# scomup/point-cloud-registration

Measured on AMD Instinct MI355X. Metric: M-correspondences/sec, plane calc_H_g_e2 on the B-01 stand-in (1.06 M pts), higher is better.
Workload: dtype f32; 1 GPU; plane_b01; kind=plane, target_points=1060000, scan_points_per_gpu=1060000, parallelism=scan-shard x1, devices_visible=1, scan_points_job=1060000, gauss_newton_iters_to_converge=5, correspondences_last_step=1060000

## Files before the change

### include/pcr.h

```cpp
#ifndef PCR_H
#define PCR_H

#include <stdint.h>

#ifdef __cplusplus
extern "C" {
#endif

#define PCR_API __attribute__((visibility("default")))

#define PCR_ABI_VERSION 5

typedef int pcr_status;
enum {
    PCR_OK = 0,
    PCR_ERR_INVALID = -1,
    PCR_ERR_HIP = -2,
    PCR_ERR_NO_TARGET = -3,
    PCR_ERR_COMM = -4,
    PCR_ERR_SINGULAR = -5,
    PCR_ERR_NOMEM = -6,
    PCR_ERR_UNSUPPORTED = -7
};

// ... 275 lines not shown
PCR_API pcr_status pcr_fgr_solo_max(pcr_context *ctx, int64_t *m_max);

#define PCR_COMPAT_M_MAX 32768
#define PCR_COMPAT_K_MAX 64
PCR_API pcr_status pcr_compat_bits(pcr_context *ctx, const float *src, const float *dst, int64_t m, double d,
                                   uint64_t *bits );
PCR_API pcr_status pcr_compat_degrees(pcr_context *ctx, const float *src, const float *dst, int64_t m, double d, int64_t *deg1 ,
                                      int64_t *deg2 );
PCR_API pcr_status pcr_compat_consensus(pcr_context *ctx, const float *src, const float *dst, int64_t m, double d, int n_seeds, int k,
                                        int64_t *deg1_or_null , int64_t *deg2_or_null , int32_t *seeds ,
                                        int32_t *members , int32_t *scores , int *n_seeds_out);

enum { PCR_K_LINEARIZE = 0, PCR_K_FINALIZE = 1, PCR_K_NN = 2, PCR_K_REDUCE = 3, PCR_K_ALLREDUCE = 4, PCR_K_CERTIFY = 5, PCR_K_COUNT = 6 };
PCR_API pcr_status pcr_profile_enable(pcr_context *ctx, int on);
PCR_API pcr_status pcr_profile_reset(pcr_context *ctx);
PCR_API pcr_status pcr_profile_read(pcr_context *ctx, int64_t launches[PCR_K_COUNT], double total_ms[PCR_K_COUNT]);
PCR_API pcr_status pcr_profile_read_n(pcr_context *ctx, int capacity, int64_t *launches, double *total_ms, int *count);
PCR_API pcr_status pcr_target_index_info(pcr_target *t, double *cell, int64_t dims[3], int64_t *occupied, int64_t *n);
PCR_API pcr_status pcr_target_index_population(pcr_target *t, int64_t *pop_max, int64_t *pop_p99, int *heavy);
PCR_API pcr_status pcr_target_index_x_order(pcr_target *t, double *xq);
PCR_API int pcr_x_order_rule(int f32_point_target, int heavy, int64_t n, int cell_bits);
PCR_API pcr_status pcr_target_index_halo(pcr_target *t, double *halo, int64_t *records);
PCR_API pcr_status pcr_target_index_halo2(pcr_target *t, double *halo, int64_t *records);
PCR_API pcr_status pcr_target_filter_band(pcr_target *t, double *band);
PCR_API pcr_status pcr_nn_counters(pcr_target *t, pcr_scan *s, const double T[16], double max_dist, double out[11]);
PCR_API pcr_status pcr_nn_counters_x(pcr_target *t, pcr_scan *s, const double T[16], double max_dist, double out[3]);
PCR_API pcr_status pcr_nn_counters_edge(pcr_target *t, pcr_scan *s, const double T[16], double max_dist, double out[9]);
PCR_API pcr_status pcr_set_variant(pcr_context *ctx, int variant);
PCR_API pcr_status pcr_get_variant(pcr_context *ctx, int *variant);
PCR_API pcr_status pcr_set_nn_mode(pcr_context *ctx, int mode);
PCR_API pcr_status pcr_set_reuse(pcr_context *ctx, int mode, double tau, double mu);
PCR_API pcr_status pcr_get_reuse(pcr_context *ctx, int *mode, double *tau, double *mu);
PCR_API pcr_status pcr_scan_reuse_stats(pcr_scan *s, double out[8]);
PCR_API pcr_status pcr_set_fuse_finalize(pcr_context *ctx, int on);
PCR_API int pcr_has_dev_kernels(void);
PCR_API pcr_status pcr_get_pipeline(pcr_context *ctx, int *variant, int *fuse_finalize, int *nn_mode);

#ifdef __cplusplus
}
#endif
#endif
```

### point_cloud_registration_amd/_capi.py

```python

import atexit
import ctypes as C
import os
import weakref

import numpy as np

_HERE = os.path.dirname(os.path.abspath(__file__))
LIB_PATH = os.environ.get("PCR_LIB") or os.path.join(_HERE, "libpcr_hip.so")
DEV_LIB_PATH = os.path.join(_HERE, "libpcr_hip_dev.so")

PCR_OK = 0
PCR_ERR_INVALID, PCR_ERR_HIP, PCR_ERR_NO_TARGET, PCR_ERR_COMM, PCR_ERR_SINGULAR, PCR_ERR_NOMEM = -1, -2, -3, -4, -5, -6
PCR_ERR_UNSUPPORTED = -7
ICP, PLANE, VPLANE, NDT = 0, 1, 2, 3
FLAG_ICP_RR_QUIRK = 1
FLAG_NO_SCAN_SORT = 2
FLAG_LOCAL_ONLY = 4
FLAG_HOST_LOOP = 8
FLAG_DEVICE_LOOP = 16
FLAG_KEEP_ORDER = 32
K_LINEARIZE, K_FINALIZE, K_NN, K_REDUCE, K_ALLREDUCE, K_CERTIFY, K_COUNT = 0, 1, 2, 3, 4, 5, 6
KERNEL_NAMES = ("linearize", "finalize", "nn", "reduce", "allreduce", "certify")
NN_FULL, NN_TRACK, NN_LIST = 0, 1, 2
# ... 66 lines not shown
    "pcr_ransac_poses": (C.c_int, [_vp, _f32p, _f32p, C.c_int64, C.c_int64, C.c_uint64, C.c_float, C.c_float, C.c_float,
                                   C.POINTER(C.c_int64), _f32p, C.POINTER(C.c_int32), C.POINTER(C.c_int64), _vp, _vp, _vp]),
    "pcr_pose_score_splits": (C.c_int, [C.c_int64, C.c_int64]),
    "pcr_fgr_linearize": (C.c_int, [_vp, _f32p, _f32p, C.c_int64, _vp, _f64p, C.c_double, _f64p, _vp]),
    "pcr_fgr_pose": (C.c_int, [_vp, _f32p, _f32p, C.c_int64, _vp, _f64p, C.c_double, C.c_double, C.c_double, C.c_int, C.c_int,
                               C.c_double, C.c_uint, _f64p, C.POINTER(C.c_int), C.POINTER(C.c_int), C.POINTER(C.c_double), _vp, _vp]),
    "pcr_fgr_tuples": (C.c_int, [_vp, _f32p, _f32p, C.c_int64, C.c_int64, C.c_uint64, C.c_float, C.c_float, _vp,
                                 C.POINTER(C.c_int64)]),
    "pcr_fgr_blocks": (C.c_int, [C.c_int64]),
    "pcr_fgr_solo_max": (C.c_int, [_vp, C.POINTER(C.c_int64)]),
    "pcr_compat_bits": (C.c_int, [_vp, _f32p, _f32p, C.c_int64, C.c_double, _vp]),
    "pcr_compat_degrees": (C.c_int, [_vp, _f32p, _f32p, C.c_int64, C.c_double, _vp, _vp]),
    "pcr_compat_consensus": (C.c_int, [_vp, _f32p, _f32p, C.c_int64, C.c_double, C.c_int, C.c_int, _vp, _vp, _vp, _vp, _vp,
                                       C.POINTER(C.c_int)]),
    "pcr_profile_enable": (C.c_int, [_vp, C.c_int]),
    "pcr_profile_reset": (C.c_int, [_vp]),
    "pcr_profile_read": (C.c_int, [_vp, _i64p, _f64p]),
    "pcr_target_index_info": (C.c_int, [_vp, C.POINTER(C.c_double), _i64p, C.POINTER(C.c_int64), C.POINTER(C.c_int64)]),
    "pcr_target_index_halo": (C.c_int, [_vp, C.POINTER(C.c_double), C.POINTER(C.c_int64)]),
    "pcr_target_index_population": (C.c_int, [_vp, C.POINTER(C.c_int64), C.POINTER(C.c_int64), C.POINTER(C.c_int)]),
    "pcr_target_index_x_order": (C.c_int, [_vp, C.POINTER(C.c_double)]),
    "pcr_x_order_rule": (C.c_int, [C.c_int, C.c_int, C.c_int64, C.c_int]),
    "pcr_set_variant": (C.c_int, [_vp, C.c_int]),
    "pcr_get_variant": (C.c_int, [_vp, C.POINTER(C.c_int)]),
    "pcr_set_nn_mode": (C.c_int, [_vp, C.c_int]),
    "pcr_set_fuse_finalize": (C.c_int, [_vp, C.c_int]),
    "pcr_get_pipeline": (C.c_int, [_vp, C.POINTER(C.c_int), C.POINTER(C.c_int), C.POINTER(C.c_int)]),
    "pcr_nn_counters": (C.c_int, [_vp, _vp, _f64p, C.c_double, _f64p]),
    "pcr_nn_counters_x": (C.c_int, [_vp, _vp, _f64p, C.c_double, _f64p]),
    "pcr_nn_counters_edge": (C.c_int, [_vp, _vp, _f64p, C.c_double, _f64p]),
    "pcr_set_reuse": (C.c_int, [_vp, C.c_int, C.c_double, C.c_double]),
    "pcr_get_reuse": (C.c_int, [_vp, C.POINTER(C.c_int), C.POINTER(C.c_double), C.POINTER(C.c_double)]),
    "pcr_scan_reuse_stats": (C.c_int, [_vp, _f64p]),
    "pcr_hash64": (C.c_int, [_vp, C.c_uint64, C.POINTER(C.c_uint64)]),
    "pcr_target_filter_band": (C.c_int, [_vp, C.POINTER(C.c_double)]),
    "pcr_target_index_halo2": (C.c_int, [_vp, C.POINTER(C.c_double), C.POINTER(C.c_int64)]),
    "pcr_usable_cpus": (C.c_int, []),
    "pcr_has_dev_kernels": (C.c_int, []),
    "pcr_abi_version": (C.c_int, []),
    "pcr_context_trim": (C.c_int, [_vp, C.POINTER(C.c_uint64)]),
    "pcr_profile_read_n": (C.c_int, [_vp, C.c_int, _i64p, _f64p, C.POINTER(C.c_int)]),
    "pcr_scan_read_matches": (C.c_int, [_vp, _vp]),
    "pcr_comm_p2p_finegrained": (C.c_int, [_vp, C.POINTER(C.c_int)]),
    "pcr_lzf_decompress": (C.c_int, [_vp, C.c_uint64, _vp, C.c_uint64, C.POINTER(C.c_uint64)]),
    "pcr_lzf_compress": (C.c_int, [_vp, C.c_uint64, _vp, C.c_uint64, C.POINTER(C.c_uint64)]),
    "pcr_gn_set": (C.c_int, [_vp, _vp, C.c_int, _vp, C.c_int, C.c_int64, C.c_int, _f64p]),
    "pcr_coreset": (C.c_int, [_vp, _f64p, C.c_int, C.c_int64, _f64p, C.c_int, C.c_int64, C.POINTER(C.c_int64), _f64p, _i64p,
                              _f64p]),
    "pcr_linearize_rows": (C.c_int, [_vp, _vp, C.c_int, _f64p, C.c_double, C.c_uint, _vp, _vp, _vp, _vp, _vp]),
    "pcr_linearize_weighted": (C.c_int, [_vp, _vp, C.c_int, _f64p, C.c_double, C.c_uint, _f64p, _f64p]),
    "pcr_scan_coreset": (C.c_int, [_vp, _vp, C.c_int, _f64p, C.c_double, C.c_uint, C.c_int, C.c_int64, _i64p, _f64p,
                                   C.POINTER(C.c_int64)]),
    "pcr_target_estimate_covariances": (C.c_int, [_vp, C.c_int, C.c_int, C.c_double, _vp]),
    "pcr_target_set_covariances": (C.c_int, [_vp, _f32p]),
    "pcr_target_get_covariances": (C.c_int, [_vp, _f32p]),
    "pcr_scan_estimate_covariances": (C.c_int, [_vp, C.c_int, C.c_int, C.c_double, _vp]),
    "pcr_scan_set_covariances": (C.c_int, [_vp, _f32p]),
    "pcr_scan_get_covariances": (C.c_int, [_vp, _f32p]),
    "pcr_gicp_linearize": (C.c_int, [_vp, _vp, _f64p, C.c_double, C.c_uint, _f64p]),
    "pcr_gicp_align": (C.c_int, [_vp, _vp, _f64p, C.c_int, C.c_double, C.c_double, C.c_uint, _f64p, C.POINTER(C.c_int), _vp]),
    "pcr_scan_estimate_normals": (C.c_int, [_vp, C.c_int, _vp]),
    "pcr_scan_set_normals": (C.c_int, [_vp, _f32p]),
    "pcr_scan_get_normals": (C.c_int, [_vp, _f32p]),
    "pcr_symm_linearize": (C.c_int, [_vp, _vp, _f64p, C.c_double, C.c_double, C.c_uint, _f64p]),
    "pcr_symm_align": (C.c_int, [_vp, _vp, _f64p, C.c_int, C.c_double, C.c_double, C.c_double, C.c_uint, _f64p, C.POINTER(C.c_int), _vp]),
    "pcr_target_set_intensity": (C.c_int, [_vp, _f32p, _vp]),
# ... 194 lines not shown

    def synchronize(self):
        check(lib().pcr_context_synchronize(self.handle))

    def stream(self):
        s = _vp()
        check(lib().pcr_context_stream(self.handle, C.byref(s)))
        return s.value

    def set_variant(self, v):
        check(lib().pcr_set_variant(self.handle, int(v)))

    def get_variant(self):
        v = C.c_int(0)
        check(lib().pcr_get_variant(self.handle, C.byref(v)))
        return v.value

    def set_nn_mode(self, m):
        check(lib().pcr_set_nn_mode(self.handle, int(m)))

    def set_fuse_finalize(self, on):
        check(lib().pcr_set_fuse_finalize(self.handle, int(bool(on))))

    def set_reuse(self, mode=None, tau=0.0, mu=0.0):
        if mode is None:
            mode = self.get_reuse()["mode"]
        check(lib().pcr_set_reuse(self.handle, int(mode), float(tau), float(mu)))

    def get_reuse(self):
        m, t, u = C.c_int(0), C.c_double(0), C.c_double(0)
        check(lib().pcr_get_reuse(self.handle, C.byref(m), C.byref(t), C.byref(u)))
        return {"mode": m.value, "tau": t.value, "mu": u.value}

    def get_pipeline(self):
        v, f, m = C.c_int(0), C.c_int(0), C.c_int(0)
        check(lib().pcr_get_pipeline(self.handle, C.byref(v), C.byref(f), C.byref(m)))
        return {"variant": v.value, "fuse_finalize": f.value, "nn_mode": m.value, "reuse": self.get_reuse()["mode"]}

    def pipeline(self, variant=None, fuse_finalize=None, nn_mode=None, reuse=None):
        import contextlib

        @contextlib.contextmanager
        def _cm():
            prev = self.get_pipeline()
            try:
                if variant is not None:
                    self.set_variant(variant)
                if fuse_finalize is not None:
                    self.set_fuse_finalize(fuse_finalize)
                if nn_mode is not None:
                    self.set_nn_mode(nn_mode)
                if reuse is not None:
                    self.set_reuse(reuse)
                yield self
            finally:
                errs = []
                for fn, val in ((self.set_variant, prev["variant"]), (self.set_fuse_finalize, prev["fuse_finalize"]),
                                (self.set_nn_mode, prev["nn_mode"]), (self.set_reuse, prev["reuse"])):
                    try:
                        fn(val)
                    except Exception as exc:
                        errs.append(exc)
                import sys as _sys
                if errs and _sys.exc_info()[0] is None:
                    raise errs[0]
        return _cm()
# ... 1196 lines not shown
```

### point_cloud_registration_amd/csrc/api.hip

```cpp
#include <math.h>
#include <stdarg.h>
#include <stdlib.h>
#include <string.h>

#include <string>

#include "gn_math.h"
#include "pcr_internal.h"

static thread_local std::string g_last_error;

void pcr_set_error(const char *fmt, ...) {
    char buf[1024];
    va_list ap;
    va_start(ap, fmt);
    vsnprintf(buf, sizeof buf, fmt, ap);
    va_end(ap);
    g_last_error = buf;
}

extern "C" const char *pcr_last_error(void) { return g_last_error.c_str(); }
extern "C" const char *pcr_version(void) { return "pcr-hip 0.4 (gfx950)"; }
extern "C" int pcr_abi_version(void) { return PCR_ABI_VERSION; }

// ... 133 lines not shown
    pcr_context *ctx = new pcr_context();
    ctx->device = device;
    ctx->num_cu = prop.multiProcessorCount > 0 ? prop.multiProcessorCount : 256;
    ctx->stream = stream;
    ctx->variant = 2;
    const char *v = getenv("PCR_VARIANT");
    if (v && *v) { const int vv = atoi(v); ctx->variant = vv == 0 ? 0 : (vv == 1 ? 1 : 2); }
    const char *nm = getenv("PCR_NN_MODE");
    if (nm && *nm) {
        const int m = atoi(nm);
#ifdef PCR_DEV
        if (m == 0 || m == 2 || m == 3 || m == 4) ctx->nn_mode = m;
#else
        if (m == 0 || m == 3) ctx->nn_mode = m;
#endif
        else fprintf(stderr, "[pcr] PCR_NN_MODE=%s is not a search mode of this library (0, 3; developer build: 2, 4): using 0\n", nm);
    }
#ifdef PCR_DEV
    const char *ff = getenv("PCR_FUSE_FINALIZE");
    if (ff && *ff) ctx->fuse_finalize = atoi(ff) != 0;
#endif
    const char *lf = getenv("PCR_LOCAL_FRAC");
    if (lf && *lf) ctx->local_frac = atof(lf);
    const char *cm = getenv("PCR_VOXEL_CELL_MULT");
    if (cm && atof(cm) > 0) ctx->voxel_cell_mult = atof(cm);
    const char *vf = getenv("PCR_VOX_FILTER");
    if (vf && *vf) ctx->vox_filter = atoi(vf) != 0;
    const char *fa = getenv("PCR_FILTER_AFTER");
    if (fa && *fa) ctx->filter_after = atoi(fa);
    const char *vo = getenv("PCR_VOX_OCC");
    if (vo && *vo) ctx->vox_occ = atoi(vo) != 0;
    const char *tl = getenv("PCR_TILE_LOCAL");
    if (tl && *tl) ctx->tile_local = atoi(tl) != 0;
    const char *sd = getenv("PCR_STALL_DEBUG");
    if (sd && *sd) ctx->stall_debug = atoi(sd) != 0;
    const char *rp = getenv("PCR_RETIRE_PERIOD");
    if (rp && *rp) ctx->retire_period = atoi(rp);
    const char *ru = getenv("PCR_REUSE");
    if (ru && *ru) ctx->reuse = atoi(ru);
    const char *rt = getenv("PCR_REUSE_TAU");
    if (rt && *rt) ctx->reuse_tau = atof(rt);
    const char *rm = getenv("PCR_REUSE_MU");
    if (rm && *rm) ctx->reuse_mu = atof(rm);
    if (ctx->reuse < 0 || ctx->reuse > 2) ctx->reuse = 0;
    const char *cl = getenv("PCR_CACHE_LIMIT_MB");
    if (cl && *cl && atof(cl) >= 0) ctx->cache_limit = (size_t)(atof(cl) * 1048576.0);
    *out = ctx;
    return PCR_OK;
}

extern "C" pcr_status pcr_context_destroy(pcr_context *ctx) {
    if (!ctx) return PCR_OK;
    (void)hipSetDevice(ctx->device);
    (void)hipStreamSynchronize(ctx->stream);
    pcr_comm_destroy(ctx);
    pcr_cache_clear(ctx);
    for (auto &e : ctx->prof_events) { (void)hipEventDestroy(e.start); (void)hipEventDestroy(e.stop); }
    for (auto &e : ctx->prof_free) { (void)hipEventDestroy(e.start); (void)hipEventDestroy(e.stop); }
    if (ctx->d_partials) (void)hipFree(ctx->d_partials);
    if (ctx->d_out) (void)hipFree(ctx->d_out);
    if (ctx->h_out) (void)hipHostFree(ctx->h_out);
    if (ctx->h_batch) (void)hipHostFree(ctx->h_batch);
    if (ctx->d_pose) (void)hipFree(ctx->d_pose);
    if (ctx->d_trace) (void)hipFree(ctx->d_trace);
    if (ctx->d_tile_ctr) (void)hipFree(ctx->d_tile_ctr);
    (void)hipStreamDestroy(ctx->stream);
    delete ctx;
    return PCR_OK;
}

extern "C" pcr_status pcr_context_trim(pcr_context *ctx, uint64_t *released_bytes) {
    PCR_REQUIRE(ctx, "ctx is NULL");
    HIP_TRY(hipSetDevice(ctx->device));
    HIP_TRY(hipStreamSynchronize(ctx->stream));
    size_t before;
    { CacheLock lock(ctx->cache_mu); before = ctx->cache_bytes; }
    pcr_cache_clear(ctx);
    if (released_bytes) *released_bytes = (uint64_t)before;
    return PCR_OK;
}

extern "C" pcr_status pcr_context_stream(pcr_context *ctx, void **stream) {
    PCR_REQUIRE(ctx && stream, "NULL argument");
    *stream = (void *)ctx->stream;
    return PCR_OK;
}

extern "C" pcr_status pcr_context_synchronize(pcr_context *ctx) {
    PCR_REQUIRE(ctx, "ctx is NULL");
    HIP_TRY(hipStreamSynchronize(ctx->stream));
    return PCR_OK;
}

extern "C" pcr_status pcr_set_variant(pcr_context *ctx, int variant) {
// ... 50 lines not shown

extern "C" pcr_status pcr_set_nn_mode(pcr_context *ctx, int mode) {
    PCR_REQUIRE(ctx, "ctx is NULL");
    PCR_REQUIRE(mode == 0 || (mode >= 2 && mode <= 4), "nn mode must be 0, 2, 3 or 4");
#ifndef PCR_DEV
    PCR_REQUIRE(mode != 2 && mode != 4, "the wave-cooperative searches (2: LDS-staged, 4: MFMA-filtered) are in the developer build only (make dev: libpcr_hip_dev.so)");
#endif
    ctx->nn_mode = mode;
    return PCR_OK;
}

extern "C" pcr_status pcr_set_reuse(pcr_context *ctx, int mode, double tau, double mu) {
    PCR_REQUIRE(ctx, "ctx is NULL");
    PCR_REQUIRE(mode >= 0 && mode <= 2, "reuse mode must be 0 (off), 1 (automatic) or 2 (forced)");
    ctx->reuse = mode;
    if (tau > 0) ctx->reuse_tau = tau;
    if (mu > 0) ctx->reuse_mu = mu;
    return PCR_OK;
}

extern "C" pcr_status pcr_get_reuse(pcr_context *ctx, int *mode, double *tau, double *mu) {
    PCR_REQUIRE(ctx, "ctx is NULL");
    if (mode) *mode = ctx->reuse;
    if (tau) *tau = ctx->reuse_tau;
    if (mu) *mu = ctx->reuse_mu;
    return PCR_OK;
}

extern "C" pcr_status pcr_scan_reuse_stats(pcr_scan *s, double out[8]) {
    PCR_REQUIRE(s && out, "NULL argument");
    out[0] = (double)s->st_passes[0]; out[1] = (double)s->st_passes[1]; out[2] = (double)s->st_passes[2];
    out[3] = (double)s->st_marked; out[4] = (double)s->st_listed_of;
    out[5] = (double)s->last_mode; out[6] = (double)s->last_marked; out[7] = s->last_motion;
    return PCR_OK;
}

#include <dlfcn.h>
static struct {
    int state;
    int (*push)(const char *);
    int (*pop)();
} g_roctx;

static bool roctx_on() {
    if (g_roctx.state == 0) {
        g_roctx.state = -1;
        const char *e = getenv("PCR_ROCTX");
        if (e && atoi(e) != 0) {
            const char *names[] = {"libroctx64.so.4", "libroctx64.so", "/opt/rocm/lib/libroctx64.so"};
            void *lib = nullptr;
            for (const char *n : names) { lib = dlopen(n, RTLD_NOW | RTLD_LOCAL); if (lib) break; }
            if (lib) {
                g_roctx.push = (int (*)(const char *))dlsym(lib, "roctxRangePushA");
                g_roctx.pop = (int (*)())dlsym(lib, "roctxRangePop");
                if (g_roctx.push && g_roctx.pop) g_roctx.state = 1;
            }
        }
    }
    return g_roctx.state == 1;
}
void pcr_roctx_push(const char *name) { if (roctx_on()) (void)g_roctx.push(name); }
void pcr_roctx_pop() { if (roctx_on()) (void)g_roctx.pop(); }

void pcr_prof_begin(pcr_context *ctx, int kernel, ProfEvent *ev) {
    ev->kernel = -1;
    if (!ctx->prof_on || !ctx->prof_this_pass) return;
// ... 583 lines not shown
```

### point_cloud_registration_amd/csrc/gn_math.h

```cpp
#pragma once

#include <math.h>

#if defined(__HIPCC__)
#define PCR_HD __host__ __device__
#else
#define PCR_HD
#endif

PCR_HD static inline int gn_solve6(double (*A)[7], const double H[36], const double g[6], double x[6]) {
#pragma unroll
    for (int i = 0; i < 6; ++i) {
#pragma unroll
        for (int j = 0; j < 6; ++j) A[i][j] = H[6 * i + j];
        A[i][6] = g[i];
    }
    int singular = 0;
#pragma unroll
    for (int c = 0; c < 6; ++c) {
        int piv = c;
        double pmax = fabs(A[c][c]);
#pragma unroll
        for (int r = c + 1; r < 6; ++r) { const double v = fabs(A[r][c]); if (v > pmax) { pmax = v; piv = r; } }
        if (pmax == 0.0) singular = 1;
// ... 111 lines not shown
    for (int k = 0; k < 7; ++k) {
        double p[3] = {(double)c[0], (double)c[1], (double)c[2]};
        if (k > 0) { const int ax = (k - 1) >> 1; p[ax] += ((k - 1) & 1) ? (double)e[ax] : -(double)e[ax]; }
        double d2 = 0;
        for (int i = 0; i < 3; ++i) {
            const double a = Ta[4 * i] * p[0] + Ta[4 * i + 1] * p[1] + Ta[4 * i + 2] * p[2] + Ta[4 * i + 3];
            const double b = Tb[4 * i] * p[0] + Tb[4 * i + 1] * p[1] + Tb[4 * i + 2] * p[2] + Tb[4 * i + 3];
            d2 += (b - a) * (b - a);
        }
        sum += sqrt(d2);
    }
    return sum / 7.0;
}

PCR_HD static inline int gn_choose_nn_mode(int reuse, int have_prev, int track_valid, double motion, double prev_motion,
                                           double tau_len) {
    if (reuse == 0 || !have_prev) return 0;
    if (reuse == 2) return track_valid ? 2 : 1;
    if (!(motion < tau_len)) return 0;
    if (track_valid) return 2;
    if (motion == 0.0) return 1;
    if (prev_motion >= 0.0 && prev_motion < 8.0 * tau_len && motion > 0.3 * prev_motion) return 1;
    return 0;
}

PCR_HD static inline double gn_filter_band(double maxabs) {
    return 1.7321 * 1.01 * maxabs * 5.9604644775390625e-8 + 1e-30;
}
PCR_HD static inline void gn_filter_bounds(double band, double bound, float *bound2_ff, float *mu_ff) {
    const double bf = (bound + band) * 1.00002;
    *bound2_ff = (float)(bf * bf * 1.000001);
    *mu_ff = (float)(2.0 * band + 3e-5 * bf);
}
```

### point_cloud_registration_amd/csrc/pass.hip

```cpp
#include <stdlib.h>

#include "pass_device.h"

static int grid8(int64_t want, int64_t cap = INT64_MAX) {
    int64_t nb = (want + 7) & ~(int64_t)7;
    if (nb > (cap & ~(int64_t)7)) nb = cap & ~(int64_t)7;
    return nb < 8 ? 8 : (int)nb;
}

static double cell_edge(const pcr_target *t) { return t->is_voxel ? t->gd.h : (double)t->gf.h; }

pcr_status pcr_ensure_scratch(pcr_context *ctx, int64_t n_points) {
    (void)n_points;
    if (!ctx->d_partials) {
        ctx->max_blocks = (ctx->num_cu * 16 + 7) & ~7;
        HIP_TRY(pcr_malloc_retry((void **)&ctx->d_partials, sizeof(double) * 32 * (size_t)(ctx->max_blocks + 8)));
        HIP_TRY(pcr_malloc_retry((void **)&ctx->d_out, sizeof(double) * 32));
        HIP_TRY(pcr_malloc_retry((void **)&ctx->d_pose, sizeof(PoseDev)));
        HIP_TRY(hipHostMalloc(&ctx->h_out, sizeof(double) * 64, hipHostMallocMapped | hipHostMallocCoherent));
        memset(ctx->h_out, 0, sizeof(double) * 64);
        HIP_TRY(hipHostGetDevicePointer((void **)&ctx->h_out_dev, ctx->h_out, 0));
        const size_t ctr_words = 9 * PCR_TICKET_STRIDE + (size_t)PCR_TILE_CTRS * PCR_TILE_STRIDE + 16;
        HIP_TRY(pcr_malloc_retry((void **)&ctx->d_tile_ctr, sizeof(uint32_t) * ctr_words));
        HIP_TRY(hipMemsetAsync(ctx->d_tile_ctr, 0, sizeof(uint32_t) * ctr_words, ctx->stream));
        auto blocks_per_cu = [](int which, int fallback) { const int nb = nn_blocks_per_cu(which); return nb > 0 ? nb : fallback; };
#ifdef PCR_DEV
        ctx->nn_blocks_per_cu[4] = blocks_per_cu(PCR_OCC_MFMA, 2);
        ctx->nn_blocks_per_cu[2] = pcr_dev_coop_blocks_per_cu();
#endif
        ctx->nn_blocks_lb = blocks_per_cu(PCR_OCC_POINT_LB, 4);
        ctx->nn_blocks_per_cu[0] = blocks_per_cu(PCR_OCC_POINT, 4);
        ctx->nn_blocks_per_cu[1] = blocks_per_cu(PCR_OCC_VOXEL, 4);
        ctx->nn_blocks_per_cu[3] = blocks_per_cu(PCR_OCC_FILTER, 4);
    }
    return PCR_OK;
}

static int64_t blocks_wanted(const pcr_context *ctx, int64_t n) {
    const int64_t want = (n + 255) / 256, cap = (int64_t)ctx->num_cu * 8;
    return want < cap ? want : cap;
}
int choose_blocks(const pcr_context *ctx, int64_t n) { return grid8(blocks_wanted(ctx, n), ctx->max_blocks); }

struct Pass {
    pcr_context *ctx;
    pcr_target *t;
    pcr_scan *s;
    int kind;
    LinArgs a;
    FinArgs f;
    bool one_kernel;
    bool fused_fin;
    bool gn_inline;
    double motion;
// ... 361 lines not shown
static pcr_status wait_host_word(pcr_context *ctx, Pred ready, const char *what) {
    for (long spin = 0; spin < 4000000L; ++spin) {
        if (ready()) { __atomic_thread_fence(__ATOMIC_ACQUIRE); return PCR_OK; }
        __builtin_ia32_pause();
    }
    HIP_TRY(hipStreamSynchronize(ctx->stream));
    if (!ready()) { pcr_set_error("%s did not report completion", what); return PCR_ERR_HIP; }
    __atomic_thread_fence(__ATOMIC_ACQUIRE);
    return PCR_OK;
}

static void retire_completed(pcr_context *ctx) {
    if (ctx->retire_period > 0 && ++ctx->passes_since_query >= (uint32_t)ctx->retire_period) {
        ctx->passes_since_query = 0;
        (void)hipStreamQuery(ctx->stream);
    }
}

pcr_status pcr_run_linearize(pcr_target *t, pcr_scan *s, int kind, const double T[16], double max_dist,
                             unsigned flags, double out[29]) {
    Pass ps;
    PCR_TRY(pass_setup(&ps, t, s, kind, max_dist, flags));
    pcr_context *ctx = ps.ctx;
    pass_set_host_pose(&ps, T);
    double motion = -1.0;
    const int mode = ps.one_kernel ? PCR_NN_FULL : host_choose_mode(&ps, T, &motion);
    ps.motion = motion;
    pass_set_mode(&ps, mode);
    const bool use_comm = ctx->comm != nullptr && !(flags & PCR_FLAG_LOCAL_ONLY);
    const bool direct = !use_comm && ctx->h_out_dev != nullptr;
    volatile uint32_t *flag = (volatile uint32_t *)(ctx->h_out + 32);
    ps.f.host_out = direct ? ctx->h_out_dev : nullptr;
    ps.f.host_flag = direct ? (volatile uint32_t *)(ctx->h_out_dev + 32) : nullptr;
    const uint32_t seq = ++ctx->seq;
    ps.f.seq = seq;
    const bool stall_dbg = ctx->stall_debug;
    struct timespec ts0, ts1, ts2, tc0, tc2;
    if (stall_dbg) { clock_gettime(CLOCK_MONOTONIC, &ts0); clock_gettime(CLOCK_THREAD_CPUTIME_ID, &tc0); }
    PCR_TRY(pass_enqueue(&ps));
    if (stall_dbg) clock_gettime(CLOCK_MONOTONIC, &ts1);
    memcpy(s->prev_T, T, sizeof s->prev_T);
    s->pose_valid = !ps.one_kernel;
    s->track_valid = mode != PCR_NN_FULL;
    s->last_mode = mode; s->last_motion = motion; s->last_marked = mode == PCR_NN_LIST ? -1 : 0;
    s->st_passes[mode] += 1;

    bool flagged = direct;
    if (use_comm) {
        ProfEvent ev;
        pcr_prof_begin(ctx, PCR_K_ALLREDUCE, &ev);
        RoctxRange range("pcr:allreduce29");
        pcr_status cs = pcr_comm_allreduce29(ctx, ctx->d_out);
        if (cs == PCR_OK && ctx->h_out_dev) {
            launch_publish(ctx->stream, ctx->d_out, ctx->h_out_dev, (volatile uint32_t *)(ctx->h_out_dev + 32), seq);
            flagged = true;
        }
        pcr_prof_end(ctx, &ev);
        if (cs != PCR_OK) return cs;
        HIP_TRY(hipGetLastError());
    }
    if (flagged) {
        PCR_TRY(wait_host_word(ctx, [&] { return *flag == seq; }, "finalize kernel"));
    } else {
        HIP_TRY(hipMemcpyAsync(ctx->h_out, ctx->d_out, sizeof(double) * 31, hipMemcpyDeviceToHost, ctx->stream));
        HIP_TRY(hipStreamSynchronize(ctx->stream));
    }
    if (use_comm && pcr_comm_failed_now(ctx)) {
        pcr_set_error("peer-to-peer exchange: a peer did not arrive (its sums were not reduced)");
        return PCR_ERR_COMM;
    }
    if (stall_dbg && flagged) {
        clock_gettime(CLOCK_MONOTONIC, &ts2); clock_gettime(CLOCK_THREAD_CPUTIME_ID, &tc2);
        const double cpu = (tc2.tv_sec - tc0.tv_sec) * 1e3 + (tc2.tv_nsec - tc0.tv_nsec) * 1e-6;
        const double enq = (ts1.tv_sec - ts0.tv_sec) * 1e3 + (ts1.tv_nsec - ts0.tv_nsec) * 1e-6;
        const double wait = (ts2.tv_sec - ts1.tv_sec) * 1e3 + (ts2.tv_nsec - ts1.tv_nsec) * 1e-6;
        if (enq + wait > 1.0) {
            fprintf(stderr, "[pcr stall] seq %u: enqueue %.3f ms, wait for the result %.3f ms; this thread was ON a CPU for %.3f ms of it\n",
                    seq, enq, wait, cpu);
        }
    }
    for (int i = 0; i < 29; ++i) out[i] = ctx->h_out[i];
    if (mode == PCR_NN_LIST && !use_comm) {
        s->last_marked = (int64_t)ctx->h_out[29];
        s->st_marked += s->last_marked; s->st_listed_of += s->n;
    }
    if (flagged) retire_completed(ctx);
    return PCR_OK;
}

static const int AHEAD = 2;
template <typename Progress, typename Enqueue>
static pcr_status drive_device_loop(pcr_context *ctx, int max_iter, int *enq, Progress &&progress, Enqueue &&enqueue, const char *stuck) {
    long spin = 0;
    for (;;) {
// ... 365 lines not shown
```

### point_cloud_registration_amd/csrc/pass_device.h

```cpp
#pragma once

#include <string.h>
#include <time.h>

#include <type_traits>

#include "gn_math.h"
#include "nn_device.h"

struct PoseK {
    float r32[9], t32[3];
    double R[9];
};
struct PoseQ {
    float r32[9], t32[3];
};

struct LinArgs {
    const float *sx, *sy, *sz;
    int64_t n;
    Geom<float> gf;
    const PtF *pts;
    uint32_t pts_last;
    const PtN *pn;
// ... 295 lines not shown
#pragma unroll
            for (int u = 0; u < W; ++u) {
                use[u] = use[u] && j[u] != PCR_NONE;
                gather_slot<KIND>(a, j[u], use[u], q[u], nr[u]);
            }
            reduce_phase();
#pragma unroll
            for (int u = 0; u < W; ++u) {
                if (!use[u]) continue;
                float tx, ty, tz;
                xform(P, x[u], y[u], z[u], tx, ty, tz);
                accumulate_point<KIND, true>(acc, a, P, q[u], nr[u], x[u], y[u], z[u], tx, ty, tz);
            }
        }
    } else {
        for (int64_t i = base; i < end; i += stride) {
            const uint32_t j = a.nn_j[i];
            if (j == PCR_NONE) continue;
            const float x = a.sx[i], y = a.sy[i], z = a.sz[i];
            float tx, ty, tz;
            xform(P, x, y, z, tx, ty, tz);
            accumulate<KIND, true>(acc, a, P, j, x, y, z, tx, ty, tz);
        }
    }
}

__device__ __forceinline__ double shfl_xor_f64(double v, int mask) {
    int lo = __double2loint(v), hi = __double2hiint(v);
    lo = __shfl_xor(lo, mask, 64);
    hi = __shfl_xor(hi, mask, 64);
    return __hiloint2double(hi, lo);
}

template <int HALF, int MASK>
__device__ __forceinline__ void fold_step(double *acc, int lane) {
    const bool upper = (lane & MASK) != 0;
#pragma unroll
    for (int i = 0; i < HALF; ++i) {
        const double send = upper ? acc[i] : acc[i + HALF];
        const double keep = upper ? acc[i + HALF] : acc[i];
        acc[i] = keep + shfl_xor_f64(send, MASK);
    }
}

__device__ __forceinline__ void wave_fold32(double *acc, int lane) {
    fold_step<16, 32>(acc, lane);
    fold_step<8, 16>(acc, lane);
    fold_step<4, 8>(acc, lane);
    fold_step<2, 4>(acc, lane);
    fold_step<1, 2>(acc, lane);
    acc[0] += shfl_xor_f64(acc[0], 1);
}

template <bool COHERENT = false>
__device__ __forceinline__ void block_store_partials(double *acc, double *__restrict__ partials) {
    __shared__ double wsum[4][32];
    const int lane = threadIdx.x & 63, wave = threadIdx.x >> 6;
    wave_fold32(acc, lane);
    if ((lane & 1) == 0) wsum[wave][lane >> 1] = acc[0];
    __syncthreads();
    if (threadIdx.x < 32) {
        const double s = ((wsum[0][threadIdx.x] + wsum[1][threadIdx.x]) + wsum[2][threadIdx.x]) + wsum[3][threadIdx.x];
        double *dst = &partials[(size_t)blockIdx.x * 32 + threadIdx.x];
        if (COHERENT) __hip_atomic_store(dst, s, __ATOMIC_RELAXED, __HIP_MEMORY_SCOPE_AGENT);
        else *dst = s;
    }
}

struct TileIter {
    int64_t base, end, stride;
    __device__ __forceinline__ TileIter(const LinArgs &a) {
        const int per = a.nblocks >> 3;
        const int xcd = (int)(blockIdx.x & 7), bi = (int)(blockIdx.x >> 3);
        const int64_t span = (((a.n + 7) >> 3) + 255) & ~(int64_t)255;
        const int64_t lo = span * xcd;
        end = lo + span < a.n ? lo + span : a.n;
        base = lo + (int64_t)bi * 256 + threadIdx.x;
        stride = (int64_t)per * 256;
    }
};

template <int HALO, int SETTLE, int B, int Q6 = 0>
__device__ __forceinline__ bool nn_filter_core(const LinArgs &a, float tx, float ty, float tz, uint32_t &w, double &d);

// ... 7 lines not shown
        uint32_t bj, bo;
        bool ok;
        if (KIND == PCR_ICP || KIND == PCR_PLANE) {
            float best;
            nn_search<float, PtF, false, false, HALO != 0, false, false, PCR_NN_BATCH_SMALL, LB>(a.gf, a.pts, a.cell_start, tx, ty, tz,
                                                                                                   a.bound2_f, best, bj, bo);
            ok = bj != PCR_NONE && __builtin_sqrtf(best) < a.md_f;
        } else if (FILT) {
            double d;
            bool cert = nn_filter_core<HALO, 1, PCR_NN_BATCH_SMALL>(a, tx, ty, tz, bj, d);
            if (!cert) {
                nn_search<double, PtD, false, false, false, false, false, PCR_NN_BATCH_SMALL>(a.gd, a.means, a.cell_start, (double)tx, (double)ty,
                                                                                           (double)tz, a.bound2_d, d, bj, bo);
            }
            ok = bj != PCR_NONE && __builtin_sqrt(d) < a.md_d;
        } else {
            double best;
            nn_search<double, PtD, false, false, false, false, false, PCR_NN_BATCH_SMALL>(a.gd, a.means, a.cell_start, (double)tx, (double)ty,
                                                                                       (double)tz, a.bound2_d, best, bj, bo);
            ok = bj != PCR_NONE && __builtin_sqrt(best) < a.md_d;
        }
        if (ok) accumulate<KIND, false>(acc, a, P, bj, x, y, z, tx, ty, tz);
    }
}

#ifndef PCR_TILE_CTRS
#define PCR_TILE_CTRS 64
#endif
#ifndef PCR_TILE_STRIDE
#define PCR_TILE_STRIDE 32
#endif
#ifndef PCR_TICKET_STRIDE
#define PCR_TICKET_STRIDE 32
#endif
#ifndef PCR_TILE_STATIC_ROUNDS
#define PCR_TILE_STATIC_ROUNDS 1
#endif
#define PCR_TILE_SUB (PCR_TILE_CTRS / 8)
#ifndef PCR_TILE_CHUNK
#define PCR_TILE_CHUNK 16
#endif
#ifndef PCR_TILE_INTERLEAVE
#define PCR_TILE_INTERLEAVE 1
#endif
template <int TP>
__device__ __forceinline__ int64_t nn_tile_real(const LinArgs &a, int xcd, int64_t lo_x, int64_t first) {
    const int64_t v = (first - lo_x) / TP;
    return (((v / PCR_TILE_CHUNK) * 8 + xcd) * PCR_TILE_CHUNK + v % PCR_TILE_CHUNK) * TP;
}

template <int LOCAL, int TP, typename Body>
__device__ __forceinline__ void nn_tile_loop(const LinArgs &a, Body &&body) {
    const int xcd = (int)(blockIdx.x & 7);
    const int lane = threadIdx.x & 63;
    const uint32_t xb = blockIdx.x >> 3, nxb = gridDim.x >> 3;
    __shared__ uint32_t blk_next;
    if (LOCAL) {
        if (threadIdx.x == 0) blk_next = 0;
        __syncthreads();
    }
#if PCR_TILE_INTERLEAVE
    {
        const int64_t chunk = (int64_t)PCR_TILE_CHUNK * TP;
        const int64_t nchunks = (a.n + chunk - 1) / chunk;
        const int64_t vspan = ((nchunks + 7) / 8) * chunk;
        if (LOCAL) {
// ... 227 lines not shown
                const double ylo_ = g.oy + (double)y * g.h;
                const double dym = fmax(fmax(ylo_ - qy, qy - (ylo_ + g.h)) - g.slack, 0.0);
                const bool live = y <= yh && dzm * dzm + dym * dym <= bd;
                const uint32_t row = (uint32_t)z * plane + (uint32_t)(live ? y : yl) * unx;
                const uint32_t s0 = cell_start[row + (uint32_t)xl] & g.cs_mask, e0 = cell_start[row + (uint32_t)xh + 1u] & g.cs_mask;
                s_[k] = s0; e_[k] = live ? e0 : s0;
            }
#pragma unroll
            for (int k = 0; k < 5; ++k) nn_scan_range<double, PtD, 0>(means, s_[k], e_[k], qx, qy, qz, bd, bj, bo);
        }
    }
}

__device__ __forceinline__ void nn_point_fix(const LinArgs &a, const PoseK &P, int64_t i, uint32_t nominee) {
    float tx, ty, tz;
    xform(P, a.sx[i], a.sy[i], a.sz[i], tx, ty, tz);
    double bd;
    uint32_t bj, bo;
    nn_box_f64(a.gd, a.means, a.cell_start, (double)tx, (double)ty, (double)tz, nominee, bd, bj, bo);
    a.nn_j[i] = __builtin_sqrt(bd) < a.md_d ? bj : PCR_NONE;
}

struct FinArgs {
    const double *partials;
    uint32_t *tile_ctr;
    uint32_t *tickets;
    int nblocks;
    int kind;
    double R[9];
    double *out;
    double *host_out;
    volatile uint32_t *host_flag;
    uint32_t seq;
    int nn_mode;
    const uint32_t *ucnt;
    int n_ucnt;
    float bb_c[3], bb_e[3];
    double local_len;
    double deep_len;
    PoseDev *pose;
    int max_iter;
    double tol;
    double *trace;
    double *host_T;
    volatile unsigned long long *host_state;
};

struct BatchItem {
    const float *sx, *sy, *sz;
    int64_t n;
    double *partials;
    uint32_t *tickets;
    PoseDev *pose;
    double *out;
    double *trace;
    double *host_T;
    unsigned long long *host_state;
    int nblocks;
    int pad;
    float bb_c[3], bb_e[3];
    double T[16];
};

template <typename T>
__device__ __forceinline__ T *uniform_ptr(T *p) {
    const unsigned long long v = (unsigned long long)p;
// ... 58 lines not shown
    block_store_partials<true>(acc, a.partials);

    __shared__ int role;
    __shared__ double part[8][33];
    __shared__ double tot[32];
    const int ng = 8;
    const int g = (int)(blockIdx.x & 7), per = f.nblocks / ng;
    uint32_t *ctr1 = &f.tickets[g * PCR_TICKET_STRIDE], *ctr2 = &f.tickets[8 * PCR_TICKET_STRIDE];
    double *rows = const_cast<double *>(f.partials);
    asm volatile("s_waitcnt vmcnt(0)" ::: "memory");
    if (threadIdx.x == 0) {
        const uint32_t t = __hip_atomic_fetch_add(ctr1, 1u, __ATOMIC_RELAXED, __HIP_MEMORY_SCOPE_AGENT);
        role = t == (uint32_t)(per - 1);
    }
    __syncthreads();
    if (!role) return false;

    const int c = threadIdx.x & 31, r0 = threadIdx.x >> 5;
    double s16[16];
#pragma unroll
    for (int u = 0; u < 16; ++u) s16[u] = 0.0;
    for (int i0 = 0; i0 < per; i0 += 128) {
#pragma unroll
        for (int u = 0; u < 16; ++u) {
            const int i = i0 + r0 + 8 * u;
            double v = 0.0;
            if (i < per) v = __hip_atomic_load(&rows[(size_t)(g + ng * i) * 32 + c], __ATOMIC_RELAXED, __HIP_MEMORY_SCOPE_AGENT);
            s16[u] += v;
        }
    }
    part[r0][c] = (((s16[0] + s16[1]) + (s16[2] + s16[3])) + ((s16[4] + s16[5]) + (s16[6] + s16[7]))) +
                  (((s16[8] + s16[9]) + (s16[10] + s16[11])) + ((s16[12] + s16[13]) + (s16[14] + s16[15])));
    __syncthreads();
    if (threadIdx.x < 32) {
        const int k = threadIdx.x;
        const double t = ((part[0][k] + part[1][k]) + (part[2][k] + part[3][k])) + ((part[4][k] + part[5][k]) + (part[6][k] + part[7][k]));
        __hip_atomic_store(&rows[(size_t)(f.nblocks + g) * 32 + k], t, __ATOMIC_RELAXED, __HIP_MEMORY_SCOPE_AGENT);
    }
    asm volatile("s_waitcnt vmcnt(0)" ::: "memory");
    if (threadIdx.x == 0) {
        __hip_atomic_store(ctr1, 0u, __ATOMIC_RELAXED, __HIP_MEMORY_SCOPE_AGENT);
        const uint32_t t2 = __hip_atomic_fetch_add(ctr2, 1u, __ATOMIC_RELAXED, __HIP_MEMORY_SCOPE_AGENT);
        role = t2 == 7u;
    }
    __syncthreads();
    if (!role) return false;

    if (threadIdx.x == 0) __hip_atomic_store(ctr2, 0u, __ATOMIC_RELAXED, __HIP_MEMORY_SCOPE_AGENT);
    if (threadIdx.x < 32) {
        double v[8];
#pragma unroll
        for (int gg = 0; gg < 8; ++gg)
            v[gg] = __hip_atomic_load(&rows[(size_t)(f.nblocks + gg) * 32 + threadIdx.x], __ATOMIC_RELAXED, __HIP_MEMORY_SCOPE_AGENT);
        tot[threadIdx.x] = ((v[0] + v[1]) + (v[2] + v[3])) + ((v[4] + v[5]) + (v[6] + v[7]));
    }
    __syncthreads();
    finalize_emit(f, tot);
    return true;
}

template <int N, typename F>
static void with_const(int v, F &&f) {
    if constexpr (N > 1) {
        if (v != N - 1) return with_const<N - 1>(v, f);
    }
    f(std::integral_constant<int, N - 1>{});
}

#define PCR_LIST_CHUNK 1024
struct FusedVariant {
    bool halo, filt, gn;
// ... 28 lines not shown
```

### point_cloud_registration_amd/csrc/pcr_internal.h

```cpp
#pragma once

#include <hip/hip_runtime.h>
#include <stdint.h>
#include <stdio.h>
#include <mutex>
#include <unordered_map>
#include <utility>
#include <vector>

#include "pcr.h"

void pcr_set_error(const char *fmt, ...);

#define HIP_TRY(expr)                                                                          \
    do {                                                                                       \
        hipError_t e_ = (expr);                                                                \
        if (e_ != hipSuccess) {                                                                \
            pcr_set_error("%s failed: %s (%s:%d)", #expr, hipGetErrorString(e_), __FILE__, __LINE__); \
            return PCR_ERR_HIP;                                                                \
        }                                                                                      \
    } while (0)

#define PCR_TRY(expr)                      \
    do {                                   \
// ... 118 lines not shown
        return e;
    }
    void reset() {
        if (p) {
            if (persist) pcr_persist_free(owner, p);
            else if (owner) pcr_cache_put(owner, p, cap);
            else (void)hipFree(p);
        }
        p = nullptr; cap = 0;
    }
    T *release() {
        T *q = p;
        p = nullptr; cap = 0;
        return q;
    }
    operator T *() const { return p; }
};

struct ProfEvent {
    int kernel;
    hipEvent_t start, stop;
};

struct pcr_context {
    int device = 0;
    int num_cu = 256;
    hipStream_t stream = nullptr;
    double *d_partials = nullptr;
    int max_blocks = 0;
    double *d_out = nullptr;
    double *h_out = nullptr;
    double *h_out_dev = nullptr;
    uint32_t seq = 0;
    uint32_t passes_since_query = 0;
    bool stall_debug = false;
    int retire_period = 0;
    PoseDev *d_pose = nullptr;
    double *d_trace = nullptr;
    int trace_cap = 0;
    char *h_batch = nullptr;
    char *h_batch_dev = nullptr;
    size_t h_batch_cap = 0;
    int variant = 0;
    int nn_mode = 0;
    double local_frac = 0.35;
    double voxel_cell_mult = 2.0;
    int vox_filter = 1;
    int filter_after = 8;
    int vox_occ = -1;
    int tile_local = -1;
    int reuse = 0;
    double reuse_tau = 0.0125;
    double reuse_mu = 0.05;
    uint64_t next_serial = 1;
    bool fuse_finalize = true;
    uint32_t *d_tile_ctr = nullptr;
    int nn_blocks_per_cu[5] = {4, 4, 4, 4, 2};
    int nn_blocks_lb = 4;
    uint32_t filter_stamp = 0;
    bool prof_on = false;
    int prof_period = 1;
    uint64_t prof_pass = 0;
    bool prof_this_pass = false;
    std::vector<ProfEvent> prof_events;
    std::vector<ProfEvent> prof_free;
    int64_t prof_launches[PCR_K_COUNT] = {0};
// ... 168 lines not shown
```

Baseline: 10190 Mcorr/s.

## Fold group partial rows on host and use DPP/permlane swaps in wave reduction

```diff
diff --git a/include/pcr.h b/include/pcr.h
--- a/include/pcr.h
+++ b/include/pcr.h
@@ -331,6 +331,7 @@
 PCR_API pcr_status pcr_set_reuse(pcr_context *ctx, int mode, double tau, double mu);
 PCR_API pcr_status pcr_get_reuse(pcr_context *ctx, int *mode, double *tau, double *mu);
 PCR_API pcr_status pcr_scan_reuse_stats(pcr_scan *s, double out[8]);
+PCR_API pcr_status pcr_context_host_fold_passes(pcr_context *ctx, uint64_t *passes);
 PCR_API pcr_status pcr_set_fuse_finalize(pcr_context *ctx, int on);
 PCR_API int pcr_has_dev_kernels(void);
 PCR_API pcr_status pcr_get_pipeline(pcr_context *ctx, int *variant, int *fuse_finalize, int *nn_mode);
diff --git a/point_cloud_registration_amd/_capi.py b/point_cloud_registration_amd/_capi.py
--- a/point_cloud_registration_amd/_capi.py
+++ b/point_cloud_registration_amd/_capi.py
@@ -122,6 +122,7 @@
     "pcr_set_reuse": (C.c_int, [_vp, C.c_int, C.c_double, C.c_double]),
     "pcr_get_reuse": (C.c_int, [_vp, C.POINTER(C.c_int), C.POINTER(C.c_double), C.POINTER(C.c_double)]),
     "pcr_scan_reuse_stats": (C.c_int, [_vp, _f64p]),
+    "pcr_context_host_fold_passes": (C.c_int, [_vp, C.POINTER(C.c_uint64)]),
     "pcr_hash64": (C.c_int, [_vp, C.c_uint64, C.POINTER(C.c_uint64)]),
     "pcr_target_filter_band": (C.c_int, [_vp, C.POINTER(C.c_double)]),
     "pcr_target_index_halo2": (C.c_int, [_vp, C.POINTER(C.c_double), C.POINTER(C.c_int64)]),
@@ -382,6 +383,11 @@
         check(lib().pcr_get_reuse(self.handle, C.byref(m), C.byref(t), C.byref(u)))
         return {"mode": m.value, "tau": t.value, "mu": u.value}
 
+    def host_fold_passes(self):
+        n = C.c_uint64(0)
+        check(lib().pcr_context_host_fold_passes(self.handle, C.byref(n)))
+        return int(n.value)
+
     def get_pipeline(self):
         v, f, m = C.c_int(0), C.c_int(0), C.c_int(0)
         check(lib().pcr_get_pipeline(self.handle, C.byref(v), C.byref(f), C.byref(m)))
diff --git a/point_cloud_registration_amd/csrc/api.hip b/point_cloud_registration_amd/csrc/api.hip
--- a/point_cloud_registration_amd/csrc/api.hip
+++ b/point_cloud_registration_amd/csrc/api.hip
@@ -189,6 +189,8 @@
     if (vo && *vo) ctx->vox_occ = atoi(vo) != 0;
     const char *tl = getenv("PCR_TILE_LOCAL");
     if (tl && *tl) ctx->tile_local = atoi(tl) != 0;
+    const char *hf = getenv("PCR_HOST_FOLD");
+    if (hf && *hf) ctx->host_fold = atoi(hf) != 0;
     const char *sd = getenv("PCR_STALL_DEBUG");
     if (sd && *sd) ctx->stall_debug = atoi(sd) != 0;
     const char *rp = getenv("PCR_RETIRE_PERIOD");
@@ -217,6 +219,7 @@
     if (ctx->d_partials) (void)hipFree(ctx->d_partials);
     if (ctx->d_out) (void)hipFree(ctx->d_out);
     if (ctx->h_out) (void)hipHostFree(ctx->h_out);
+    if (ctx->h_rows) (void)hipHostFree(ctx->h_rows);
     if (ctx->h_batch) (void)hipHostFree(ctx->h_batch);
     if (ctx->d_pose) (void)hipFree(ctx->d_pose);
     if (ctx->d_trace) (void)hipFree(ctx->d_trace);
@@ -333,6 +336,12 @@
     out[0] = (double)s->st_passes[0]; out[1] = (double)s->st_passes[1]; out[2] = (double)s->st_passes[2];
     out[3] = (double)s->st_marked; out[4] = (double)s->st_listed_of;
     out[5] = (double)s->last_mode; out[6] = (double)s->last_marked; out[7] = s->last_motion;
+    return PCR_OK;
+}
+
+extern "C" pcr_status pcr_context_host_fold_passes(pcr_context *ctx, uint64_t *passes) {
+    PCR_REQUIRE(ctx && passes, "NULL argument");
+    *passes = ctx->host_fold_passes;
     return PCR_OK;
 }
 
diff --git a/point_cloud_registration_amd/csrc/gn_math.h b/point_cloud_registration_amd/csrc/gn_math.h
--- a/point_cloud_registration_amd/csrc/gn_math.h
+++ b/point_cloud_registration_amd/csrc/gn_math.h
@@ -167,3 +167,11 @@
     *bound2_ff = (float)(bf * bf * 1.000001);
     *mu_ff = (float)(2.0 * band + 3e-5 * bf);
 }
+
+PCR_HD static inline void gn_fold8_rows(const volatile double *rows, double *tot, int ncomp) {
+    for (int k = 0; k < ncomp; ++k) {
+        const double v0 = rows[k], v1 = rows[32 + k], v2 = rows[64 + k], v3 = rows[96 + k];
+        const double v4 = rows[128 + k], v5 = rows[160 + k], v6 = rows[192 + k], v7 = rows[224 + k];
+        tot[k] = ((v0 + v1) + (v2 + v3)) + ((v4 + v5) + (v6 + v7));
+    }
+}
diff --git a/point_cloud_registration_amd/csrc/pass.hip b/point_cloud_registration_amd/csrc/pass.hip
--- a/point_cloud_registration_amd/csrc/pass.hip
+++ b/point_cloud_registration_amd/csrc/pass.hip
@@ -7,6 +7,8 @@
     if (nb > (cap & ~(int64_t)7)) nb = cap & ~(int64_t)7;
     return nb < 8 ? 8 : (int)nb;
 }
+
+#define PCR_HOST_ROWS_BYTES (sizeof(double) * 8 * 32 + sizeof(uint32_t) * 8 * PCR_GFLAG_STRIDE)
 
 static double cell_edge(const pcr_target *t) { return t->is_voxel ? t->gd.h : (double)t->gf.h; }
 
@@ -20,6 +22,9 @@
         HIP_TRY(hipHostMalloc(&ctx->h_out, sizeof(double) * 64, hipHostMallocMapped | hipHostMallocCoherent));
         memset(ctx->h_out, 0, sizeof(double) * 64);
         HIP_TRY(hipHostGetDevicePointer((void **)&ctx->h_out_dev, ctx->h_out, 0));
+        HIP_TRY(hipHostMalloc((void **)&ctx->h_rows, PCR_HOST_ROWS_BYTES, hipHostMallocMapped | hipHostMallocCoherent));
+        memset(ctx->h_rows, 0, PCR_HOST_ROWS_BYTES);
+        HIP_TRY(hipHostGetDevicePointer((void **)&ctx->h_rows_dev, ctx->h_rows, 0));
         const size_t ctr_words = 9 * PCR_TICKET_STRIDE + (size_t)PCR_TILE_CTRS * PCR_TILE_STRIDE + 16;
         HIP_TRY(pcr_malloc_retry((void **)&ctx->d_tile_ctr, sizeof(uint32_t) * ctr_words));
         HIP_TRY(hipMemsetAsync(ctx->d_tile_ctr, 0, sizeof(uint32_t) * ctr_words, ctx->stream));
@@ -447,8 +452,16 @@
     volatile uint32_t *flag = (volatile uint32_t *)(ctx->h_out + 32);
     ps.f.host_out = direct ? ctx->h_out_dev : nullptr;
     ps.f.host_flag = direct ? (volatile uint32_t *)(ctx->h_out_dev + 32) : nullptr;
-    const uint32_t seq = ++ctx->seq;
+    if (++ctx->seq == 0) ctx->seq = 1;
+    const uint32_t seq = ctx->seq;
     ps.f.seq = seq;
+    const bool host_fold = direct && ctx->host_fold && ctx->h_rows_dev != nullptr && ps.fused_fin && kind != PCR_ICP && mode != PCR_NN_LIST;
+    volatile uint32_t *gflags = (volatile uint32_t *)(ctx->h_rows + 8 * 32);
+    if (host_fold) {
+        ps.f.host_rows = ctx->h_rows_dev;
+        ps.f.host_gflags = (volatile uint32_t *)(ctx->h_rows_dev + 8 * 32);
+        ctx->host_fold_passes += 1;
+    }
     const bool stall_dbg = ctx->stall_debug;
     struct timespec ts0, ts1, ts2, tc0, tc2;
     if (stall_dbg) { clock_gettime(CLOCK_MONOTONIC, &ts0); clock_gettime(CLOCK_THREAD_CPUTIME_ID, &tc0); }
@@ -474,7 +487,15 @@
         if (cs != PCR_OK) return cs;
         HIP_TRY(hipGetLastError());
     }
-    if (flagged) {
+    if (host_fold) {
+        auto all_groups = [&] {
+            for (int g = 0; g < 8; ++g)
+                if (gflags[g * PCR_GFLAG_STRIDE] != seq) return false;
+            return true;
+        };
+        PCR_TRY(wait_host_word(ctx, all_groups, "the fold of a group"));
+        gn_fold8_rows(ctx->h_rows, ctx->h_out, 29);
+    } else if (flagged) {
         PCR_TRY(wait_host_word(ctx, [&] { return *flag == seq; }, "finalize kernel"));
     } else {
         HIP_TRY(hipMemcpyAsync(ctx->h_out, ctx->d_out, sizeof(double) * 31, hipMemcpyDeviceToHost, ctx->stream));
diff --git a/point_cloud_registration_amd/csrc/pass_device.h b/point_cloud_registration_amd/csrc/pass_device.h
--- a/point_cloud_registration_amd/csrc/pass_device.h
+++ b/point_cloud_registration_amd/csrc/pass_device.h
@@ -351,14 +351,62 @@
     return __hiloint2double(hi, lo);
 }
 
+#ifndef PCR_FOLD_SWAP
+#define PCR_FOLD_SWAP 1
+#endif
+#if PCR_FOLD_SWAP && defined(__has_builtin)
+#if __has_builtin(__builtin_amdgcn_permlane32_swap) && __has_builtin(__builtin_amdgcn_permlane16_swap) && __has_builtin(__builtin_amdgcn_update_dpp)
+#define PCR_FOLD_SWAP_ON 1
+#endif
+#endif
+#ifndef PCR_FOLD_SWAP_ON
+#define PCR_FOLD_SWAP_ON 0
+#endif
+
+#if PCR_FOLD_SWAP_ON
+#define PCR_DPP_ROW_ROR8 0x128
+#define PCR_DPP_QUAD_XOR2 0x4E
+#define PCR_DPP_QUAD_XOR1 0xB1
+template <int CTRL>
+__device__ __forceinline__ double dpp_f64(double v) {
+    const int lo = __double2loint(v), hi = __double2hiint(v);
+    return __hiloint2double(__builtin_amdgcn_update_dpp(hi, hi, CTRL, 0xf, 0xf, false),
+                            __builtin_amdgcn_update_dpp(lo, lo, CTRL, 0xf, 0xf, false));
+}
+#endif
+
+template <int MASK>
+__device__ __forceinline__ double xchg_f64(double v) {
+#if PCR_FOLD_SWAP_ON
+    if constexpr (MASK == 8) return dpp_f64<PCR_DPP_ROW_ROR8>(v);
+    else if constexpr (MASK == 2) return dpp_f64<PCR_DPP_QUAD_XOR2>(v);
+    else if constexpr (MASK == 1) return dpp_f64<PCR_DPP_QUAD_XOR1>(v);
+    else
+#endif
+    return shfl_xor_f64(v, MASK);
+}
+
 template <int HALF, int MASK>
 __device__ __forceinline__ void fold_step(double *acc, int lane) {
+#if PCR_FOLD_SWAP_ON
+    if constexpr (MASK == 32 || MASK == 16) {
+#pragma unroll
+        for (int i = 0; i < HALF; ++i) {
+            const unsigned alo = (unsigned)__double2loint(acc[i]), ahi = (unsigned)__double2hiint(acc[i]);
+            const unsigned blo = (unsigned)__double2loint(acc[i + HALF]), bhi = (unsigned)__double2hiint(acc[i + HALF]);
+            const auto lo = MASK == 32 ? __builtin_amdgcn_permlane32_swap(alo, blo, false, false) : __builtin_amdgcn_permlane16_swap(alo, blo, false, false);
+            const auto hi = MASK == 32 ? __builtin_amdgcn_permlane32_swap(ahi, bhi, false, false) : __builtin_amdgcn_permlane16_swap(ahi, bhi, false, false);
+            acc[i] = __hiloint2double((int)hi[0], (int)lo[0]) + __hiloint2double((int)hi[1], (int)lo[1]);
+        }
+        return;
+    }
+#endif
     const bool upper = (lane & MASK) != 0;
 #pragma unroll
     for (int i = 0; i < HALF; ++i) {
         const double send = upper ? acc[i] : acc[i + HALF];
         const double keep = upper ? acc[i + HALF] : acc[i];
-        acc[i] = keep + shfl_xor_f64(send, MASK);
+        acc[i] = keep + xchg_f64<MASK>(send);
     }
 }
 
@@ -368,7 +416,7 @@
     fold_step<4, 8>(acc, lane);
     fold_step<2, 4>(acc, lane);
     fold_step<1, 2>(acc, lane);
-    acc[0] += shfl_xor_f64(acc[0], 1);
+    acc[0] += xchg_f64<1>(acc[0]);
 }
 
 template <bool COHERENT = false>
@@ -442,6 +490,7 @@
 #endif
 #ifndef PCR_TICKET_STRIDE
 #define PCR_TICKET_STRIDE 32
+#define PCR_GFLAG_STRIDE 16
 #endif
 #ifndef PCR_TILE_STATIC_ROUNDS
 #define PCR_TILE_STATIC_ROUNDS 1
@@ -735,6 +784,8 @@
     double *host_out;
     volatile uint32_t *host_flag;
     uint32_t seq;
+    double *host_rows;
+    volatile uint32_t *host_gflags;
     int nn_mode;
     const uint32_t *ucnt;
     int n_ucnt;
@@ -859,11 +910,26 @@
     part[r0][c] = (((s16[0] + s16[1]) + (s16[2] + s16[3])) + ((s16[4] + s16[5]) + (s16[6] + s16[7]))) +
                   (((s16[8] + s16[9]) + (s16[10] + s16[11])) + ((s16[12] + s16[13]) + (s16[14] + s16[15])));
     __syncthreads();
+    double t = 0.0;
     if (threadIdx.x < 32) {
         const int k = threadIdx.x;
-        const double t = ((part[0][k] + part[1][k]) + (part[2][k] + part[3][k])) + ((part[4][k] + part[5][k]) + (part[6][k] + part[7][k]));
-        __hip_atomic_store(&rows[(size_t)(f.nblocks + g) * 32 + k], t, __ATOMIC_RELAXED, __HIP_MEMORY_SCOPE_AGENT);
-    }
+        t = ((part[0][k] + part[1][k]) + (part[2][k] + part[3][k])) + ((part[4][k] + part[5][k]) + (part[6][k] + part[7][k]));
+    }
+    if (f.host_rows != nullptr) {
+        if (threadIdx.x < 32) {
+            f.host_rows[g * 32 + threadIdx.x] = t;
+            __threadfence_system();
+        }
+        __syncthreads();
+        if (threadIdx.x == 0) {
+            f.host_gflags[g * PCR_GFLAG_STRIDE] = f.seq;
+            __hip_atomic_store(ctr1, 0u, __ATOMIC_RELAXED, __HIP_MEMORY_SCOPE_AGENT);
+        }
+        if (g == 0 && threadIdx.x < PCR_TILE_CTRS) f.tile_ctr[threadIdx.x * PCR_TILE_STRIDE] = 0;
+        return false;
+    }
+    if (threadIdx.x < 32)
+        __hip_atomic_store(&rows[(size_t)(f.nblocks + g) * 32 + threadIdx.x], t, __ATOMIC_RELAXED, __HIP_MEMORY_SCOPE_AGENT);
     asm volatile("s_waitcnt vmcnt(0)" ::: "memory");
     if (threadIdx.x == 0) {
         __hip_atomic_store(ctr1, 0u, __ATOMIC_RELAXED, __HIP_MEMORY_SCOPE_AGENT);
diff --git a/point_cloud_registration_amd/csrc/pcr_internal.h b/point_cloud_registration_amd/csrc/pcr_internal.h
--- a/point_cloud_registration_amd/csrc/pcr_internal.h
+++ b/point_cloud_registration_amd/csrc/pcr_internal.h
@@ -174,6 +174,9 @@
     double *h_out = nullptr;
     double *h_out_dev = nullptr;
     uint32_t seq = 0;
+    double *h_rows = nullptr, *h_rows_dev = nullptr;
+    bool host_fold = true;
+    uint64_t host_fold_passes = 0;
     uint32_t passes_since_query = 0;
     bool stall_debug = false;
     int retire_period = 0;
```

Measured after the change: 10400 Mcorr/s, median of 6. 2.0% higher.
